# nihofm/volren

Measured on AMD Instinct MI355X. Metric: Msamples/s (pixels x spp / s), volume path tracing, higher is better.
Workload: dtype f32; 1 GPU; BASELINE configs[1] 'c2': smoke.brick, no transfer function, 1024x1024, 1024 spp, seed 42, fov 40; parallelism=1 GPU, 1 fused launch(es)/frame (sample pool budget 64 GiB)

## Files before the change

### volren_amd/csrc/capi.cpp

```cpp
#include "../../include/volren_amd.h"

#include <algorithm>
#include <cmath>
#include <cstring>
#include <filesystem>
#include <functional>
#include <iostream>
#include <stdexcept>
#include <memory>
#include <string>
#include <vector>

#include "imageio.h"
#include "renderer.h"
#include "sharded.h"
#include "vr_device.h"
#include "vr_math_probe.h"

struct vr_renderer {
    vr::RendererHIP impl;
    int device = 0;
};

struct vr_sharded {
// ... 242 lines not shown
    return guard([&] {
        auto& R = r->impl;
        const std::string n = name;
        if (n == "sample") { R.sample = v; R.drop_tile_samples(); }
        else if (n == "sppx") R.sppx = v;
        else if (n == "seed") R.seed = v;
        else if (n == "bounces") R.bounces = v;
        else if (n == "show_environment") R.show_environment = v != 0;
        else if (n == "tonemapping") R.tonemapping = v != 0;
        else if (n == "integrator") R.integrator = v;
        else if (n == "fast_math") R.fast_math = v != 0;
        else if (n == "variance") { if (v < 0 || v > 1) throw std::runtime_error("variance: 0 (off) or 1 (keep the per-pixel second moments)"); R.variance = v; }
        else if (n == "denoise_iterations") {
            if (v < 0 || v > vr::kDenoiseMaxIterations) throw std::runtime_error("denoise_iterations must be in [0, 10]");
            R.denoise_iterations = v;
        }
        else if (n == "denoise_moments") R.set_denoise_moments(v);
        else if (n == "denoise_resolve") R.set_denoise_resolve(v);
        else if (n == "denoise_layers") R.set_denoise_layers(v);
        else if (n == "coalesce_trace") { R.flush_pending(); R.coalesce_trace = v != 0; }
        else if (n == "majorant_layout") { if (v < -1 || v > 1) throw std::runtime_error("majorant_layout: -1 (per grid, chosen at commit), 0 (linear), 1 (4x4x4-cell blocks)"); R.majorant_layout = v; }
        else if (n == "tf_float_atlas") R.tf_float_atlas = v != 0;
        else if (n == "wide_addressing") { if (v < 0 || v > 1) throw std::runtime_error("wide_addressing: 0 (by the tables' sizes), 1 (always the kernels with 64-bit gather addresses)"); R.tuning.wide_addressing = v; }
        else if (n == "gpu_encoder") R.gpu_encoder = v != 0;
        else if (n == "sample_pool_mb") { if (v < 16 || v > 65536) throw std::runtime_error("sample_pool_mb must be in [16, 65536] (item indices of a sub-launch are 32-bit: < 2^32 RGBA32F items)"); R.sample_pool_bytes = (size_t)v << 20; }
        else if (n == "seed_table_mb") {
            if (v < -1 || v > vr::RendererHIP::kSeedTableMaxMb) throw std::runtime_error("seed_table_mb must be in [0, 8192] (0 = no table), or -1 for the default min(4096, sample_pool_mb / 4)");
            R.seed_table_mb = v;
        }
        else if (n == "seed_table_max_samples") { if (v < 0) throw std::runtime_error("seed_table_max_samples must be >= 0 (0 = as many as seed_table_mb holds)"); R.seed_table_max_samples = v; }
        else if (n == "launch_target_ms") { if (v < 0) throw std::runtime_error("launch_target_ms must be >= 0 (0 = no sizing by time)"); R.launch_target_ms = v; }
        else if (n == "expected_skip") { if (v < 0 || v > 1) throw std::runtime_error("expected_skip: 0 (march every step) or 1 (drop the steps of empty space by the clear-distance table)"); R.expected_skip = v; }
        else if (n == "expected_stats") { if (v < 0 || v > 1) throw std::runtime_error("expected_stats: 0 (off) or 1 (the expected-value passes count their work)"); R.expected_stats = v; }
        else if (n == "order_tiles") { if (v < 0 || v > 2) throw std::runtime_error("order_tiles: 0 (never), 1 (tile subsets), 2 (always)"); R.order_tiles = v; }
        else if (n == "grid_frame_counter") {
            if (!R.volume || v < 0 || (size_t)v >= R.volume->n_grid_frames()) throw std::runtime_error("grid_frame_counter out of range");
            R.volume->grid_frame_counter = (size_t)v;
        } else throw std::runtime_error("unknown int parameter: " + n);
    });
}

int vr_get_int(vr_renderer* r, const char* name, int* v) {
    NEED(r);
    if (!name || !v) return fail(VR_ERR_ARG, "null argument");
    return guard([&] {
        auto& R = r->impl;
// ... 2 lines not shown
        else if (n == "sppx") *v = R.sppx;
        else if (n == "seed") *v = R.seed;
        else if (n == "bounces") *v = R.bounces;
        else if (n == "show_environment") *v = R.show_environment ? 1 : 0;
        else if (n == "tonemapping") *v = R.tonemapping ? 1 : 0;
        else if (n == "integrator") *v = R.integrator;
        else if (n == "fast_math") *v = R.fast_math ? 1 : 0;
        else if (n == "variance") *v = R.variance;
        else if (n == "denoise_iterations") *v = R.denoise_iterations;
        else if (n == "denoise_moments") *v = R.denoise_moments;
        else if (n == "denoise_resolve") *v = R.denoise_resolve;
        else if (n == "denoise_layers") *v = R.denoise_layers;
        else if (n == "coalesce_trace") *v = R.coalesce_trace ? 1 : 0;
        else if (n == "majorant_layout") *v = R.majorant_layout;
        else if (n == "majorant_blocked") {
            vr::SceneParams P; R.fill_params(P); *v = P.density.maj_blocked;
        }
        else if (n == "kernel_variant" || n == "kernel_variant_reason") {
            vr::SceneParams P; R.fill_params(P);
            int why = 0; const int variant = vr::pathtrace_variant_of(P, &why);
            *v = n == "kernel_variant" ? variant : why;
        }
        else if (n == "wide_addressing") *v = R.tuning.wide_addressing;
        else if (n == "kernel_wide") {
            vr::SceneParams P; R.fill_params(P);
            *v = (vr::pathtrace_wide_of(R.tuning, P) || vr::pathtrace_variant_of(P, nullptr) >= 2) ? 1 : 0;
        }
        else if (n == "env_div_safe") *v = R.environment && R.environment->cdf_div_safe ? 1 : 0;
        else if (n == "env_compact") *v = R.environment && R.environment->envmap_rgbe ? 1 : 0;
        else if (n == "pending_samples") *v = R.pending_samples();
        else if (n == "tf_float_atlas") *v = R.tf_float_atlas ? 1 : 0;
        else if (n == "gpu_encoder") *v = R.gpu_encoder ? 1 : 0;
        else if (n == "sample_pool_mb") *v = (int)(R.sample_pool_bytes >> 20);
        else if (n == "seed_table_mb") *v = R.seed_table_budget_mb();
        else if (n == "seed_table_max_samples") *v = R.seed_table_max_samples;
        else if (n == "seed_table_samples") *v = R.seed_table_samples();
        else if (n == "seed_table_fills") *v = R.seed_table_fills();
        else if (n == "launch_target_ms") *v = R.launch_target_ms;
        else if (n == "expected_skip") *v = R.expected_skip;
        else if (n == "expected_stats") *v = R.expected_stats;
        else if (n == "order_tiles") *v = R.order_tiles;
        else if (n == "grid_frame_counter") *v = R.volume ? (int)R.volume->grid_frame_counter : 0;
        else if (n == "n_grid_frames") *v = R.volume ? (int)R.volume->n_grid_frames() : 0;
        else if (n == "last_launches") *v = R.last_launches;
        else if (n == "adaptive_rounds") *v = R.adaptive_rounds;
        else if (n == "width") *v = R.resolution.x;
// ... 497 lines not shown
```

### volren_amd/csrc/renderer.cpp

```cpp
#include "renderer.h"

#include <algorithm>
#include <cfloat>
#include <cmath>
#include <cstdlib>
#include <cstring>
#include <iostream>
#include <mutex>

#include "vr_adaptive.h"
#include "vr_device.h"
#include "vr_math.h"
#include "vr_probe.h"

namespace vr {

mat3 Camera::view_inverse() const {
    const vec3 f = normalize(dir);
    const vec3 s = normalize(cross(f, up));
    const vec3 u = cross(s, f);
    mat3 r(0.0f);
    r.m[0] = s.x; r.m[1] = s.y; r.m[2] = s.z;
    r.m[3] = u.x; r.m[4] = u.y; r.m[5] = u.z;
    r.m[6] = -f.x; r.m[7] = -f.y; r.m[8] = -f.z;
    return r;
}

RendererHIP::~RendererHIP() {
    if (ev0_) (void)hipEventDestroy(ev0_);
    if (ev1_) (void)hipEventDestroy(ev1_);
    for (hipEvent_t e : pt_events_) (void)hipEventDestroy(e);
    if (seed_event_) (void)hipEventDestroy(seed_event_);
}

void RendererHIP::init() {
    int n_dev = 0;
    if (hipGetDeviceCount(&n_dev) != hipSuccess || n_dev == 0)
        throw std::runtime_error("RendererHIP::init: no HIP device available (this renderer has no CPU path)");
    if (!volume) volume = std::make_shared<Volume>();
    if (!environment) {
        const float white[3] = { 1.f, 1.f, 1.f };
        environment = std::make_shared<Environment>(white, 1, 1);
    }
    if (!ev0_) { VR_HIP(hipEventCreate(&ev0_)); VR_HIP(hipEventCreate(&ev1_)); }
    if (!status_) {
        status_ = make_device_buffer(16 * sizeof(uint32_t));
        VR_HIP(hipMemset(status_->get(), 0, 16 * sizeof(uint32_t)));
    }
    if (!color && resolution.x > 0 && resolution.y > 0) resize((uint32_t)resolution.x, (uint32_t)resolution.y);
}

void RendererHIP::resize(uint32_t w, uint32_t h) {
    if (w == 0 || h == 0) throw std::runtime_error("RendererHIP::resize: empty framebuffer");
    pending_n_ = 0; pending_ = LaunchInputs{};
    resolution = { (int)w, (int)h };
    color = make_device_buffer((size_t)w * h * 4 * sizeof(float));
    display.reset();
    sized_ = Sized{};
    drop_tile_samples();
    drop_seed_table();
    VR_HIP(hipMemset(color->get(), 0, color->size_bytes()));
    if (!tiles_host_.empty()) set_tiles(tiles_host_);
}

void RendererHIP::reset() { sample = 0; drop_tile_samples(); }

static void check_grid_bytes(size_t bytes, const char* what, const int32_t nb[3]);
constexpr size_t kBlockedMajorantBricks = (size_t)1 << 18;
static size_t brick_records(const BrickGridHIP& g);

// ... 381 lines not shown
    for (size_t k = 0; k < ids.size(); ++k) ordered[k] = ids[(size_t)perm[k]];
    return ordered;
}

const int32_t* RendererHIP::tile_order(const SceneParams& P, const std::vector<int32_t>& ids, int n_tiles) {
    const Uniforms& u = P.u;
    uint64_t key = 1469598103934665603ull;
    auto mix = [&key](const void* p, size_t nbytes) { const uint8_t* b = static_cast<const uint8_t*>(p); for (size_t i = 0; i < nbytes; ++i) { key ^= b[i]; key *= 1099511628211ull; } };
    mix(u.cam_pos, sizeof u.cam_pos); mix(u.cam_transform, sizeof u.cam_transform); mix(&P.cam_z, sizeof P.cam_z);
    mix(u.vol_bb_min, sizeof u.vol_bb_min); mix(u.vol_bb_max, sizeof u.vol_bb_max); mix(u.resolution, sizeof u.resolution); mix(&n_tiles, sizeof n_tiles);
    if (!ids.empty()) mix(ids.data(), ids.size() * sizeof(int32_t));
    key = key ? key : 1;
    if (order_dev_ && order_key_ == key && order_dev_->size_bytes() == (size_t)n_tiles * sizeof(int32_t)) return order_dev_->as<int32_t>();
    const std::vector<int32_t> ordered = costliest_first(P, ids, n_tiles);
    ensure_buffer(order_dev_, ordered.size() * sizeof(int32_t));
    order_dev_->upload(ordered.data(), ordered.size() * sizeof(int32_t), stream);
    order_key_ = key;
    return order_dev_->as<int32_t>();
}

bool RendererHIP::LaunchInputs::same_launch_as(const LaunchInputs& o) const {
    return memcmp(&P, &o.P, sizeof P) == 0 && frame == o.frame && maj.density_scale == o.maj.density_scale && maj.tf_version == o.maj.tf_version &&
           maj.wl == o.maj.wl && maj.ww == o.maj.ww && maj.blocked == o.maj.blocked && memcmp(tuning.thr, o.tuning.thr, sizeof tuning.thr) == 0 && tuning.stats == o.tuning.stats &&
           tuning.samples_per_unit == o.tuning.samples_per_unit && tuning.blocks_per_cu == o.tuning.blocks_per_cu && tuning.wide_addressing == o.tuning.wide_addressing && order_tiles == o.order_tiles &&
           launch_target_ms == o.launch_target_ms && fast_math == o.fast_math && variance == o.variance && sample_pool_bytes == o.sample_pool_bytes && stream == o.stream;
}

void RendererHIP::capture(LaunchInputs& in) {
    if (!color) throw std::runtime_error("RendererHIP::trace: no framebuffer (call resize first)");
    if (integrator == 2 && !transferfunc) throw std::runtime_error("RendererHIP::trace: integrator 2 (direct volume rendering) needs a transfer function");
    if (integrator < 0 || integrator > 3) throw std::runtime_error("RendererHIP::trace: unknown integrator");
    if (fast_math && transferfunc) throw std::runtime_error("RendererHIP::trace: fast_math is not available while a transfer function is bound (it misses the 1e-3 bound there); set fast_math 0");
    if (!volume || volume->grids.empty() || density_grids.empty()) throw std::runtime_error("RendererHIP::trace: no volume committed");
    if (volume->grid_frame_counter >= density_grids.size()) throw std::runtime_error("RendererHIP::trace: grid_frame_counter out of range (commit() after changing the volume)");
    {
        BrickGridHIP& g = density_grids[volume->grid_frame_counter];
        const bool build = transferfunc && tf_float_atlas && !g.dense && g.atlas && g.rng && !g.atlas_f32 && !g.atlas_f32_failed;
        const bool drop = (!transferfunc || !tf_float_atlas) && (g.atlas_f32 || g.atlas_f32_failed);
        if (build || drop) flush_pending();
        if (build) {
            try {
                const size_t n_blocks = g.atlas->size_bytes() / kBrickBlockBytes, want = n_blocks * 512u * sizeof(float);
                auto drop_others = [&] { for (BrickGridHIP& other : density_grids) if (&other != &g) other.atlas_f32.reset(); };
                size_t free_b = 0, total_b = 0;
                if (hipMemGetInfo(&free_b, &total_b) != hipSuccess) { (void)hipGetLastError(); free_b = ~(size_t)0; }
                if (want > free_b / 2) drop_others();
                try { g.atlas_f32 = make_device_buffer(want); }
// ... 111 lines not shown
            if (first > 0) sized_.moments_n = -1;
        }
        moments = sized_.moments->as<float>();
        sized_.moments_n = first == 0 ? n : (sized_.moments_n == first ? first + n : -1);
    } else {
        sized_.moments_n = -1;
    }
    if (!keep_timing_) {
        VR_HIP(hipEventRecord(ev0_, stream));
        last_launches = 0;
        pt_events_used_ = 0;
    }
    for (int done = 0; done < n;) {
        ++last_launches;
        const int m = probe > 0 ? probe : std::min(per_launch, n - done);
        hipEvent_t eb = nullptr, ee = nullptr;
        if (pt_kernel) {
            while (pt_events_.size() < pt_events_used_ + 2) { hipEvent_t e; VR_HIP(hipEventCreate(&e)); pt_events_.push_back(e); }
            eb = pt_events_[pt_events_used_]; ee = pt_events_[pt_events_used_ + 1];
            pt_events_used_ += 2;
        }
        int seed_samples = 0;
        const uint32_t* seed_table = pathtrace_reads_seed_table(in.tuning, P) ? seed_table_for(P, first + done, m, stream, &seed_samples) : nullptr;
        launch_pathtrace(in.tuning, P, color->as<float>(), pool_->as<float>(), workspace_->as<float>(), status_->as<uint32_t>() + 1, tiles, n_tiles, first + 1 + done, m, status_->as<uint32_t>(), stream, in.fast_math != 0, eb, ee, moments,
                         seed_table, seed_samples);
        VR_HIP(hipGetLastError());
        done += m;
        if (pt_kernel) { rate_pending_samples_ = px_samples * (double)m; rate_pending_key_ = key; }
        if (probe > 0) {
            probe = 0;
            harvest_rate(true);
            per_launch = cap_by_rate(per_launch);
        }
    }
    VR_HIP(hipEventRecord(ev1_, stream));
    timing_pending_ = true;
}

int RendererHIP::seed_table_samples_for(long long mb, int w, int h) {
    if (mb <= 0 || w <= 0 || h <= 0) return 0;
    const long long per_sample = (long long)tile_count(w, h) * 256 * (long long)sizeof(uint32_t);
    return (int)std::min<long long>((mb << 20) / per_sample, 1 << 24);
}

void RendererHIP::drop_seed_table() {
    seed_table_.reset();
    seed_cap_ = seed_filled_ = 0;
// ... 626 lines not shown
```

### volren_amd/csrc/renderer.h

```cpp
#pragma once

#include <algorithm>
#include <memory>
#include <string>
#include <vector>

#include "devmem.h"
#include "environment.h"
#include "grids.h"
#include "transferfunc.h"
#include "vr_device.h"
#include "vr_scene.h"

namespace vr {

struct Camera {
    vec3 pos{ 1.f, 0.f, 1.f };
    vec3 dir = normalize(-pos);
    vec3 up{ 0.f, 1.f, 0.f };
    float fov_degree = 70.f;
    mat3 view_inverse() const;
};

struct BrickGridHIP {
// ... 156 lines not shown
        size_t sample_pool_bytes = 0;
        hipStream_t stream = nullptr;
        std::shared_ptr<Environment> env;
        std::shared_ptr<TransferFunction> tf;
        DeviceBufferPtr keep[5];
        bool same_launch_as(const LaunchInputs& o) const;
    };
    void capture(LaunchInputs& in);
    void submit(const LaunchInputs& in, int first, int n, const int32_t* tiles, int n_tiles);
    void submit_tile_set(const LaunchInputs& in, int first, int n);
    int samples_per_launch(const LaunchInputs& in, int n_tiles) const;
    LaunchInputs pending_;
    int pending_n_ = 0, pending_first_ = 0, pending_cap_ = 0;
    void update_majorants(const LaunchInputs& in, BrickGridHIP& g);
    std::vector<int32_t> tiles_host_;
    DeviceBufferPtr tiles_dev_;
    DeviceBufferPtr order_dev_;
    uint64_t order_key_ = 0;
    std::vector<int32_t> costliest_first(const SceneParams& P, const std::vector<int32_t>& ids, int n_tiles) const;
    const int32_t* tile_order(const SceneParams& P, const std::vector<int32_t>& ids, int n_tiles);
    std::vector<int32_t> tile_n_;
    int tile_n_sample_ = -1;
    bool keep_timing_ = false;
    DeviceBufferPtr status_;
    DeviceBufferPtr pool_;
    DeviceBufferPtr workspace_;
    DeviceBufferPtr seed_table_;
    int seed_cap_ = 0, seed_filled_ = 0, seed_fills_ = 0, seed_budget_mb_ = -1, seed_max_samples_ = 0;
    int seed_key_[3] = { 0, 0, 0 };
    bool seed_failed_ = false;
    hipStream_t seed_stream_ = nullptr;
    hipEvent_t seed_event_ = nullptr;
    void drop_seed_table();
    const uint32_t* seed_table_for(const SceneParams& P, int s0, int n, hipStream_t stream, int* samples);
    DeviceBufferPtr stats_;
    struct Sized {
        DeviceBufferPtr features;
        int pass = 0, rays = 0;
        DeviceBufferPtr moments;
        int moments_n = -1;
        DeviceBufferPtr rs_bg, rs_part, resolved;
        DeviceBufferPtr ly_split, ly_filtered, layer;
        bool layer_valid = false;
        DeviceBufferPtr dn_guide, dn_var[2], dn_color[2];
        DeviceBufferPtr denoised;
        DeviceBufferPtr dn_reject;
// ... 34 lines not shown
```

### volren_amd/csrc/vr_device.h

```cpp
#pragma once

#include <hip/hip_runtime.h>
#include <stdint.h>

#include "vr_denoise.h"
#include "vr_scene.h"
#include "vr_temporal.h"
#include "vr_tiles.h"

namespace vr {

struct PathtraceTuning {
    int32_t thr[8] = { 64, 0, 56, 0, 60, 60, 64, 0 };
    unsigned long long* stats = nullptr;
    int32_t samples_per_unit = 0;
    int32_t blocks_per_cu = 0;
    int32_t wide_addressing = 0;
};
PathtraceTuning default_tuning();
size_t pathtrace_pool_floats(const PathtraceTuning& T, int32_t n_tiles, int32_t n_samples);
size_t pathtrace_workspace_floats();
void launch_pathtrace(const PathtraceTuning& T, const SceneParams& P, float* fb, float* sample_pool, float* workspace, uint32_t* unit_counter, const int32_t* tiles, int32_t n_tiles,
                      int32_t first_sample, int32_t n_samples, uint32_t* status, hipStream_t stream, bool fast_math = false,
                      hipEvent_t ev_kernel_begin = nullptr, hipEvent_t ev_kernel_end = nullptr,
                      float* moments = nullptr,
                      const uint32_t* seed_table = nullptr, int32_t seed_samples = 0);
constexpr uint32_t kFeatureLostStatus = 4u;
void launch_features(const SceneParams& P, const int32_t* tiles, int32_t n_tiles, int32_t spp, float* out, uint32_t* status, hipStream_t stream);
constexpr int32_t kExpectedMaxRays = 4;
void launch_features_expected(const SceneParams& P, const int32_t* tiles, int32_t n_tiles, int32_t rays, float* out, hipStream_t stream,
                              const ClearTable* clear = nullptr, unsigned long long* stats = nullptr);
enum PathtraceVariantReason : int {
    VR_VARIANT_INTEGRATOR = 1,
    VR_VARIANT_ENV_DIVISION = 2,
    VR_VARIANT_DENSITY_SCALE = 4,
    VR_VARIANT_GRID_FORMS = 8
};
int pathtrace_variant_of(const SceneParams& P, int* why);
bool pathtrace_reads_seed_table(const PathtraceTuning& T, const SceneParams& P);
bool pathtrace_wide_of(const PathtraceTuning& T, const SceneParams& P);
void launch_denoise_prepare(const float* moments, const float* features, int32_t W, int32_t H, int32_t n, float vscale, const int32_t* counts, float* v, float* guide,
                            hipStream_t stream);
void launch_denoise_atrous(const float* cin, const float* vin, const float* guide, int32_t W, int32_t H, int32_t step, const DenoiseSigma& sg,
                           float* cout, float* vout, hipStream_t stream);
// ... 51 lines not shown
```

### volren_amd/csrc/vr_launch.hip

```cpp
#include <hip/hip_runtime.h>

#include <algorithm>
#include <cstdlib>
#include <map>
#include <mutex>
#include <stdexcept>
#include <string>

#include "vr_device.h"
#include "vr_expected.h"
#include "vr_pathtrace.h"

namespace vr {

template <int INTEGRATOR>
__global__ void __launch_bounds__(256)
item_kernel(const SceneParams P, float* __restrict__ sbuf, const LaunchDesc D) {
    const uint32_t per_unit = (uint32_t)(D.spu * 64);
    const uint32_t g = blockIdx.x * 256u + threadIdx.x;
    const uint32_t u = g / per_unit, item = g - u * per_unit;
    if (u >= D.n_units) return;
    const WorkUnit wu = make_unit(D, P.u.resolution[0], u, sbuf);
    if ((int32_t)item >= wu.n_items) return;
    const int32_t px = wu.px0 + (int32_t)(item & 7u), py = wu.py0 + (int32_t)((item >> 3) & 7u);
// ... 179 lines not shown
    }
    return variant;
}

static int resident_blocks(const PathtraceTuning& T, int mode, int wide, int variant, bool tf, bool stats) {
    int dev = 0, cus = 0;
    if (hipGetDevice(&dev) != hipSuccess) return 1024;
    static std::mutex mu;
    static std::map<uint32_t, std::pair<int, int>> cache;
    const uint32_t key = ((uint32_t)dev << 8) | ((uint32_t)wide << 6) | ((uint32_t)mode << 5) | ((uint32_t)variant << 2) | (tf ? 2u : 0u) | (stats ? 1u : 0u);
    std::pair<int, int> v;
    {
        std::lock_guard<std::mutex> lock(mu);
        auto it = cache.find(key);
        if (it == cache.end()) {
            if (hipDeviceGetAttribute(&cus, hipDeviceAttributeMultiprocessorCount, dev) != hipSuccess || cus <= 0) cus = 256;
            it = cache.emplace(key, std::make_pair(cus, kPtOccupancy[mode][wide][variant](tf, stats))).first;
        }
        v = it->second;
    }
    const int per_cu = T.blocks_per_cu > 0 ? T.blocks_per_cu : v.second;
    return std::min(v.first * per_cu, kMaxWorkgroups * 4 / kWgWaves);
}

size_t pathtrace_workspace_floats() { return kColdMainFloats + (size_t)kMaxWorkgroups * 4u * (size_t)kColdSideWaveFloats; }

void launch_pathtrace(const PathtraceTuning& T, const SceneParams& P, float* fb, float* sample_pool, float* workspace, uint32_t* unit_counter, const int32_t* tiles, int32_t n_tiles,
                      int32_t first_sample, int32_t n_samples, uint32_t* status, hipStream_t stream, bool fast_math, hipEvent_t ev_kernel_begin, hipEvent_t ev_kernel_end,
                      float* moments, const uint32_t* seed_table, int32_t seed_samples) {
    if (n_tiles <= 0 || n_samples <= 0) return;
    SchedParams S;
    for (int i = 0; i < ST_COUNT; ++i) S.thr[i] = T.thr[i];
    LaunchDesc D;
    D.tiles = tiles; D.n_tiles = n_tiles; D.first_sample = first_sample; D.n_samples = n_samples;
    const int variant = pathtrace_variant(P);
    D.spu = std::min(n_samples, samples_per_unit(T, variant));
    const int32_t chunks = (n_samples + D.spu - 1) / D.spu;
    if ((uint64_t)chunks * (uint64_t)n_tiles * 4u * (uint64_t)(D.spu * 64) > 0xFFFFFFFFull)
        throw std::runtime_error("launch_pathtrace: " + std::to_string(n_tiles) + " tiles x " + std::to_string(n_samples) + " samples do not fit the 32-bit item index of one launch");
    D.n_units = (uint32_t)chunks * (uint32_t)n_tiles * 4u;
    D.chunks = (uint32_t)chunks;
    D.seg_len = (D.n_units + kQueueSegments - 1u) / kQueueSegments;
    D.unit_counter = unit_counter;
    SeedTable seeds;
    seeds.table = seed_samples > 0 ? seed_table : nullptr;
    seeds.cap = seed_samples;
    seeds.n_tiles = tile_count(P.u.resolution[0], P.u.resolution[1]);
    S.max_iters = kMaxIdleIters;
    if (S.thr[ST_COLLIDE] <= 0) S.thr[ST_COLLIDE] = (P.u.use_tf || P.u.has_emission) ? 32 : 24;
    const bool tf = P.u.use_tf != 0, stats = T.stats != nullptr;
    const int mode = fast_math ? 1 : 0, wide = pathtrace_wide_of(T, P) ? 1 : 0;
    const int blocks = resident_blocks(T, mode, wide, variant, tf, stats);
    const uint32_t groups_needed = (D.n_units + (uint32_t)kWgWaves - 1u) / (uint32_t)kWgWaves;
    const dim3 grid((unsigned)std::min<uint32_t>((uint32_t)blocks, groups_needed > 0 ? groups_needed : 1u)), block(256);
    if (P.u.integrator == 3 || (P.u.integrator == 2 && P.u.use_tf)) {
        const uint64_t items = (uint64_t)D.n_units * (uint64_t)(D.spu * 64);
        const auto integrate = P.u.integrator == 2 ? item_kernel<2> : item_kernel<3>;
        hipLaunchKernelGGL(integrate, dim3((unsigned)((items + 255) / 256)), block, 0, stream, P, sample_pool, D);
    } else {
        (void)hipMemsetAsync(unit_counter, 0, kQueueSegments * sizeof(uint32_t), stream);
        if (ev_kernel_begin) (void)hipEventRecord(ev_kernel_begin, stream);
        kPtLaunch[mode][wide][variant](tf, stats, grid.x, stream, &P, sample_pool, workspace, &D, &S, status, T.stats, &seeds);
        if (ev_kernel_end) (void)hipEventRecord(ev_kernel_end, stream);
    }
    const auto accumulate = moments ? accumulate_kernel<true> : accumulate_kernel<false>;
    hipLaunchKernelGGL(accumulate, dim3((unsigned)n_tiles), block, 0, stream, sample_pool, fb, moments, tiles, n_tiles, P.u.resolution[0], P.u.resolution[1],
                       first_sample, n_samples, D.spu);
}

}
```

### volren_amd/csrc/vr_pathtrace.h

```cpp
#pragma once

#include <hip/hip_runtime.h>

#include <type_traits>

#include "vr_tiles.h"
#include "vr_trace.h"

namespace vr {

struct SchedParams {
    int32_t thr[ST_COUNT];
    uint32_t max_iters;
};

constexpr uint32_t kQueueSegments = 8u;
constexpr uint32_t kMaxIdleIters = 1u << 26;
constexpr uint64_t kMaxIdleTicks = 7200000000ull;
struct LaunchDesc {
    const int32_t* tiles;
    int32_t n_tiles, first_sample, n_samples, spu;
    uint32_t n_units, chunks, seg_len;
    uint32_t* unit_counter;
};
struct SeedTable {
    const uint32_t* table;
    int32_t cap, n_tiles;
};

__device__ __forceinline__ WorkUnit make_unit(const LaunchDesc& D, int32_t W, uint32_t j, float* sbuf) {
    const uint32_t rem = j / D.chunks, chunk = j - rem * D.chunks;
    const uint32_t slot = rem >> 2, sub = rem & 3u;
    const TilePixel q = wave_tiled_pixel(D.tiles ? D.tiles[slot] : (int32_t)slot, sub * 64u, W);
    WorkUnit wu;
    wu.px0 = q.px;
    wu.py0 = q.py;
    wu.first_sample = D.first_sample + (int32_t)chunk * D.spu;
    wu.n_items = min(D.spu, D.n_samples - (int32_t)chunk * D.spu) * 64;
    wu.base = pool_slot<uint32_t>(chunk, D.n_tiles, slot, sub, D.spu, 0u, 0u);
// ... 9 lines not shown
#endif
#ifndef VR_PRIO_HOT
#define VR_PRIO_HOT 1
#endif
#ifndef VR_PRIO_EVENTS
#define VR_PRIO_EVENTS 0
#endif

typedef __attribute__((address_space(1))) uint32_t SeedGlobal;
template <class K, bool STATS> constexpr int seed_request_point() {
#ifdef VR_SEED_REQ
    return VR_SEED_REQ;
#else
    if (K::emission != 0 || K::global != 0 || K::dense != 0 || STATS) return -1;
    return K::tf ? 0 : 2;
#endif
}

template <class K, bool STATS> constexpr bool collide_tail_early() {
#ifdef VR_COLLIDE_EARLY
    return K::global == 0 && VR_COLLIDE_EARLY != 0;
#else
    return !K::tf && K::global == 0 && K::emission == 0 && K::dense == 0 && K::a32 && !VR_FAST_DEVICE && !STATS;
#endif
}

constexpr int32_t kWgWaves = 4;
constexpr int32_t kLdsPerWorkgroup = 163840 / 16 * kWgWaves;
constexpr int32_t kLutLdsEntries = 256;

enum PoolStack : int32_t { Q_READY = 0, Q_NEE = 1, Q_POST = 2, Q_ESC = 3, Q_FREE = 4, Q_COUNT = 5 };

template <class K> constexpr bool lazy_emission() { return K::emission == 1; }
template <class K> constexpr int32_t hot_stride() { return lazy_emission<K>() ? 15 : 12; }
constexpr int32_t HOT_EL = 12;
template <class K> constexpr int32_t pool_slots() {
#ifdef VR_NSLOT
    return VR_NSLOT;
#else
    const int32_t shared = K::tf ? kLutLdsEntries * 16 + 16 : kWgWaves * 256;
    const int32_t n = (kLdsPerWorkgroup - shared) / kWgWaves / (hot_stride<K>() * 4 + Q_COUNT);
    return n > 192 ? 192 : n;
#endif
}
constexpr int32_t NSLOT = 192;
constexpr int32_t HOT_COL = 4;
// ... 310 lines not shown
        VR_SECTION(0);
#if !VR_STAT_SCHED
        if (STATS_T) { stat_add(26, (uint32_t)popc(wave_ballot(slot >= 0))); stat_add(27, (uint32_t)cnt_ready); stat_add(28, (uint32_t)cnt_nee); stat_add(29, (uint32_t)cnt_post); stat_add(30, (uint32_t)cnt_esc); stat_add(31, (uint32_t)cnt_free); }
#endif
#ifndef VR_HOT_PAIRS
#define VR_HOT_PAIRS 4
#endif
        constexpr int kHotPairs = VR_HOT_PAIRS;

#ifndef VR_HOT_PAIR_MIN
#define VR_HOT_PAIR_MIN 44
#endif
#ifndef VR_DRAIN
#define VR_DRAIN 0
#endif
        const uint64_t holds_path = wave_ballot(slot >= 0);
#ifndef VR_CLEAN_FORMS
#define VR_CLEAN_FORMS 1
#endif
        constexpr bool kCleanForms = VR_CLEAN_FORMS != 0;
        const bool all_clean = kCleanForms && (holds_path & wave_ballot((int32_t)f2u(l.far) < 0)) == 0ull;
        auto hot_pair = [&](auto clean_tag, const int hot_rep_) __attribute__((always_inline)) -> bool {
            constexpr bool CLEAN = decltype(clean_tag)::value;
            if (hot_rep_ > 0 && popc_s(holds_path & wave_ballot((uint32_t)(l.state - ST_MARCH) < 2u)) < (VR_DRAIN && exhausted ? 1 : VR_HOT_PAIR_MIN)) return false;
            if (STATS_T) t_blk = (uint32_t)__builtin_readcyclecounter();
            const bool is_m = slot >= 0 && l.state == ST_MARCH;
            MarchIO mio;
            march_idle(mio);
            if (is_m) march_prep<K::dense, K::majb, CLEAN>(l, P, mio);
            if constexpr (K::maj_reuse) march_load_reuse<K::tf, K::a32>(P, mio, l);
            else march_load<K::tf, K::a32>(P, mio);
            asm volatile("" : "+v"(mio.maj1), "+v"(mio.maj2));
            if (is_m) march_finish<K::tf, K::maj_reuse, CLEAN>(l, P, mio);
            if (STATS) { const int32_t nm = popc(wave_ballot(is_m)); if (nm) { stat_add(2 * ST_MARCH, 1u); stat_add(2 * ST_MARCH + 1, (uint32_t)nm); } }
            if (STATS_T) { const uint32_t t_now = (uint32_t)__builtin_readcyclecounter(); stat_add(18 + ST_MARCH, t_now - t_blk); t_blk = t_now; }
            const bool is_c = slot >= 0 && l.state == ST_COLLIDE;
            const int32_t n_c = popc(holds_path & wave_ballot(l.state == ST_COLLIDE));
            const int32_t n_m = popc(holds_path & wave_ballot(l.state == ST_MARCH));
            const bool run_c = n_c > 0 && n_c >= min(VR_THR_COLLIDE, (n_c + n_m + 1) >> 1);
            if (run_c) {
                CollideIO<K> cio;
                collide_idle<K>(cio);
                const SceneParams& PE = K::emission != 0 ? event_args().P : P;
                const SceneParams& PF = (K::tf && (K::global == 2 || K::emission == 1)) ? event_args().P : P;
                if (is_c) collide_prep<K, CLEAN>(l, PF, PE, cio);
                collide_load<K>(PF, PE, cio);
// ... 50 lines not shown
        const bool want_nee = cnt_nee > 0 && (cnt_nee >= VR_THR_NEE || (hungry && (cnt_nee == big || drain_all)));
        const bool want_post = cnt_post > 0 && (cnt_post >= VR_THR_POST || (hungry && (cnt_post == big || drain_all)));
        const bool want_esc = cnt_esc > 0 && (cnt_esc >= VR_THR_ESC || (hungry && (cnt_esc == big || drain_all)));
        if (want_new || want_nee || want_post || want_esc) {
#if VR_BATCH_REGS
            Hot b;
#else
            const int32_t my_slot = slot;
            const float my_majorant = l.majorant;
            if (my_slot >= 0) { hs.save(l, my_slot); if (emission_on && !l.shadow) { ColdT c = VR_COLD(my_slot); st3(c, C_L, l.eL); } }
            __builtin_amdgcn_wave_barrier();
            Hot& b = l;
#endif
            if (VR_PRIO_EVENTS != VR_PRIO_HOT) __builtin_amdgcn_s_setprio(VR_PRIO_EVENTS);
            constexpr int kSeedReq = seed_request_point<K, STATS>();
            auto pull_unit = [&]() __attribute__((always_inline)) {
                if (cursor != (uint32_t)wu.n_items) return;
                const KernelArgs& E = event_args();
                uint32_t j = 0xFFFFFFFFu;
                while (seg_tries < kQueueSegments) {
                    const uint32_t k = ((blockIdx.x & (kQueueSegments - 1u)) + seg_tries) & (kQueueSegments - 1u);
                    const uint32_t lo = k * E.D.seg_len, hi = min(lo + E.D.seg_len, E.D.n_units);
                    uint32_t v = 0xFFFFFFFFu;
                    if (lo < hi) { if (lane == 0) v = atomicAdd(E.D.unit_counter + k, 1u); v = __builtin_amdgcn_readfirstlane(v); }
                    if (lo < hi && v < hi - lo) { j = lo + v; break; }
                    ++seg_tries;
                }
                if (j == 0xFFFFFFFFu) { exhausted = true; if (STATS_T) t_exhausted = __builtin_amdgcn_s_memrealtime(); }
                else { wu = make_unit(E.D, E.P.u.resolution[0], j, nullptr); cursor = 0u; idle_iters = 0u; t_elapsed = 0u; }
            };
            auto seed_entry = [&](const KernelArgs& E, bool& have) __attribute__((always_inline)) -> uint32_t {
                const uint32_t item = cursor + (uint32_t)lane;
                const uint32_t s = (uint32_t)(wu.first_sample - 1) + (item >> 6);
                have = kSeedReq >= 0 && E.seeds.table != nullptr && item < (uint32_t)wu.n_items && s < (uint32_t)E.seeds.cap;
                return seed_table_index<uint32_t>(s, E.seeds.n_tiles, (uint32_t)tile_of_pixel(wu.px0, wu.py0, E.P.u.resolution[0]), sub_of_pixel(wu.px0, wu.py0), item & 63u);
            };
            auto seed_load = [&](const KernelArgs& E) __attribute__((always_inline)) -> uint32_t {
                uint32_t v = 0u;
                if (kSeedReq >= 0 && E.seeds.table != nullptr) {
                    bool have;
                    const uint32_t i = seed_entry(E, have);
                    v = *(const SeedGlobal*)(E.seeds.table + (size_t)(have ? i : (uint32_t)lane));
                    asm volatile("" ::: "memory");
                }
                return v;
            };
            uint32_t seed_early = 0u;
            auto new_batch = [&]() __attribute__((always_inline)) {
                if (want_new) {
                    if (kSeedReq != 1) pull_unit();
                    n = min(min(64, cnt_free), (int32_t)((uint32_t)wu.n_items - cursor));
                    if (n > 0) {
                        VR_STAT(ST_NEW, n);
                        int32_t bs = -1;
                        const KernelArgs& E = event_args();
                        bool have_seed;
                        seed_entry(E, have_seed);
                        uint32_t table_seed;
                        if (kSeedReq == 1) table_seed = seed_early;
                        else if (kSeedReq == 2) { table_seed = seed_next; have_seed = have_seed && seed_next_valid; }
                        else table_seed = seed_load(E);
                        if (lane < n) {
                            bs = q[Q_FREE * NS + cnt_free - 1 - lane];
                            hot_init(b);
                            ColdT c = VR_COLD(bs);
                            do_new<K, ColdT, kLazyEm>(b, c, E.P, wu, cursor + (uint32_t)lane, have_seed, table_seed);
                            hs.save_new(b, bs);
                            if (kLazyEm) hs.save_first_radiance(v3{ 0.0f, 0.0f, 0.0f }, bs);
                        }
                        cnt_free -= n;
                        cursor += (uint32_t)n;
                        VR_ROUTE_B(bs);
                        VR_STAT_END(ST_NEW);
                    }
                    if (kSeedReq == 2) { pull_unit(); seed_next = seed_load(event_args()); seed_next_valid = true; }
                }
            };
            if (kSeedReq == 1 && want_new) { pull_unit(); seed_early = seed_load(event_args()); }
            if (want_esc) {
                n = min(64, cnt_esc);
                VR_STAT(ST_ESCAPE, n);
                int32_t bs = -1;
                if (lane < n) { bs = q[Q_ESC * NS + cnt_esc - 1 - lane]; hs.load(b, bs); if (kLazyEm && b.first) b.eL = hs.load_first_radiance(bs); }
                if (kItemInRegs) b.item = item_fetch(banks, lane, bs);
                if (lane < n) {
                    const ColdT c = VR_COLD(b.first ? 0 : bs);
                    const KernelArgs& E = event_args();
                    WorkUnit w; w.out = E.sbuf;
                    do_escape<ColdT, kItemInRegs, kLazyEm, kWorld>(b, c, E.P, w);
                }
                cnt_esc -= n;
                VR_ROUTE_B(bs);
                VR_STAT_END(ST_ESCAPE);
            }
            if (want_post) {
                n = min(64, cnt_post);
                VR_STAT(ST_POSTNEE, n);
                int32_t bs = -1;
                if (lane < n) { bs = q[Q_POST * NS + cnt_post - 1 - lane]; hs.load(b, bs); }
                if (kShleInRegs) b.shle = shle_fetch(banks, lane, bs);
                if (kItemInRegs) b.item = item_fetch(banks, lane, bs);
                if (lane < n) {
                    ColdT c = VR_COLD(bs);
                    const KernelArgs& E = event_args();
                    WorkUnit w; w.out = E.sbuf;
                    do_postnee<K, ColdT, kShleInRegs, kItemInRegs>(b, c, E.P, w);
                    hs.save(b, bs);
                }
                cnt_post -= n;
                VR_ROUTE_B(bs);
                VR_STAT_END(ST_POSTNEE);
            }
            if constexpr (kSeedReq < 0) {
                if (want_new) {
                    if (cursor == (uint32_t)wu.n_items) {
                        const KernelArgs& E = event_args();
                        uint32_t j = 0xFFFFFFFFu;
                        while (seg_tries < kQueueSegments) {
                            const uint32_t k = ((blockIdx.x & (kQueueSegments - 1u)) + seg_tries) & (kQueueSegments - 1u);
                            const uint32_t lo = k * E.D.seg_len, hi = min(lo + E.D.seg_len, E.D.n_units);
                            uint32_t v = 0xFFFFFFFFu;
                            if (lo < hi) { if (lane == 0) v = atomicAdd(E.D.unit_counter + k, 1u); v = __builtin_amdgcn_readfirstlane(v); }
                            if (lo < hi && v < hi - lo) { j = lo + v; break; }
                            ++seg_tries;
                        }
                        if (j == 0xFFFFFFFFu) { exhausted = true; if (STATS_T) t_exhausted = __builtin_amdgcn_s_memrealtime(); }
                        else { wu = make_unit(E.D, E.P.u.resolution[0], j, nullptr); cursor = 0u; idle_iters = 0u; t_elapsed = 0u; }
                    }
                    n = min(min(64, cnt_free), (int32_t)((uint32_t)wu.n_items - cursor));
                    if (n > 0) {
                        VR_STAT(ST_NEW, n);
                        int32_t bs = -1;
                        if (lane < n) {
                            bs = q[Q_FREE * NS + cnt_free - 1 - lane];
                            hot_init(b);
                            ColdT c = VR_COLD(bs);
                            do_new<K, ColdT, kLazyEm>(b, c, event_args().P, wu, cursor + (uint32_t)lane);
                            hs.save_new(b, bs);
                            if (kLazyEm) hs.save_first_radiance(v3{ 0.0f, 0.0f, 0.0f }, bs);
                        }
                        cnt_free -= n;
                        cursor += (uint32_t)n;
                        VR_ROUTE_B(bs);
                        VR_STAT_END(ST_NEW);
                    }
// ... 68 lines not shown
```

### volren_amd/csrc/vr_trace.h

```cpp
#pragma once

#include <type_traits>

#include "vr_math.h"
#include "vr_scene.h"

#if defined(VR_HOST_TRACE) && !defined(__HIP_DEVICE_COMPILE__)
namespace vr {
enum TraceClass : int32_t { TR_MAJORANT = 0, TR_TAP = 1, TR_ENV_WARP = 2, TR_ENV_TEXEL = 3 };
void host_trace(int32_t cls, const void* table, size_t a, size_t b);
}
#define VR_TRACE(CLS, TABLE, A, B) ::vr::host_trace((CLS), (TABLE), (size_t)(A), (size_t)(B))
#else
#define VR_TRACE(CLS, TABLE, A, B) do { } while (0)
#endif

namespace vr {

enum LaneState : int32_t {
    ST_NEW = 0,
    ST_BEGIN = 1,
    ST_MARCH = 2,
    ST_COLLIDE = 3,
    ST_NEE = 4,
// ... 1124 lines not shown
    const uint32_t n_paths = f2u(q_l.b) + 1u;
    if (n_paths >= (uint32_t)P.u.bounces) { write_sample(wu, ITEM_IN_HOT ? h.item : ldu(c, C_ITEM), L, n_paths); h.state = ST_NEW; return; }
    const float rr = luma(thr);
    if (rr < 0.1f) {
        const float prob = 1.0f - rr;
        if (rng(h.seed) < prob) { write_sample(wu, ITEM_IN_HOT ? h.item : ldu(c, C_ITEM), L, n_paths); h.state = ST_NEW; return; }
        thr = thr / (1.0f - prob);
        if (!WS) { st3(c, C_THR, thr); c.st(C_FPL, fpl_kept); }
    }
    const v3 dir = q_d.a;
    const float s0 = rng(h.seed), s1 = rng(h.seed);
    const v3 sd = sample_phase_hg(dir, P.u.vol_phase_g, s0, s1);
    const float f_p_next = phase_hg(dot(-dir, sd), P.u.vol_phase_g);
    if (WS) {
        st3(c, C_L, L); stu(c, C_NPATHS, n_paths);
        st3(c, C_THR, thr); c.st(C_FP, f_p_next);
    } else {
        st3(c, C_L, L); stu(c, C_NPATHS, n_paths);
        st3(c, C_DIR, sd); c.st(C_FP, f_p_next);
    }
    begin_segment<K>(h, P, q_p.a, sd, 0);
}

template <class Cold, bool ITEM_IN_HOT = false, bool FIRST_L_IN_HOT = false, bool WS = false>
VR_HD void do_escape(Hot& h, const Cold& c, const SceneParams& P, const WorkUnit& wu) {
    const bool first = h.first != 0;
    v3 L = ld3(c, C_L), thr = ld3(c, C_THR), dir = ld3(c, C_DIR);
    uint32_t n_paths = ldu(c, C_NPATHS), item = ITEM_IN_HOT ? h.item : ldu(c, C_ITEM);
    const float f_p = c.ld(C_FP);
    v3 Le_early = v3{ 0.0f, 0.0f, 0.0f };
    if (WS && P.u.show_environment > 0) Le_early = lookup_environment(P, h.wdir);
    const v3 L_first = FIRST_L_IN_HOT ? h.eL : v3{ 0.0f, 0.0f, 0.0f };
    L = v3{ first ? L_first.x : L.x, first ? L_first.y : L.y, first ? L_first.z : L.z };
    thr = v3{ first ? 1.0f : thr.x, first ? 1.0f : thr.y, first ? 1.0f : thr.z };
    if (WS) dir = h.wdir;
    else dir = v3{ first ? h.ipos.x : dir.x, first ? h.ipos.y : dir.y, first ? h.ipos.z : dir.z };
    n_paths = first ? 0u : n_paths;
    item = first ? f2u(h.Tr) : item;
    h.first = 0;
    if (P.u.show_environment > 0) {
        const v3 Le = WS ? Le_early : lookup_environment(P, dir);
        float mis = 1.0f;
        if (n_paths > 0u) {
            const float avg_w = env_average_importance(P);
            const float pdf_env = (luma(Le) / avg_w) * kInv4Pi;
            mis = power_heuristic(f_p, pdf_env);
        }
        L = L + (thr * mis) * Le;
// ... 234 lines not shown
```

### volren_amd/renderer.py

```python
import ctypes as C

import numpy as np

from . import _lib

_INT_FIELDS = ("sample", "sppx", "seed", "bounces", "show_environment", "tonemapping", "integrator", "grid_frame_counter",
               "sample_pool_mb", "gpu_encoder", "fast_math", "tf_float_atlas", "launch_target_ms", "order_tiles", "coalesce_trace", "majorant_layout",
               "variance", "denoise_iterations", "denoise_moments", "denoise_resolve", "denoise_layers", "wide_addressing", "seed_table_mb", "seed_table_max_samples",
               "expected_skip", "expected_stats")
_FLOAT_FIELDS = {"tonemap_exposure": 1, "tonemap_gamma": 1, "albedo": 3, "phase": 1, "density_scale": 1,
                 "emission_scale": 1, "vol_clip_min": 3, "vol_clip_max": 3, "env_strength": 1, "env_transform": 9,
                 "tf_window_left": 1, "tf_window_width": 1, "cam_pos": 3, "cam_dir": 3, "cam_up": 3, "cam_fov": 1,
                 "volume_transform": 16, "denoise_sigma": 5, "denoise_alpha": 1, "denoise_reject": 1}


def _f32(a):
    return np.ascontiguousarray(a, dtype=np.float32)


class Renderer:

    def __init__(self, width, height, device=0, _borrowed=None):
        object.__setattr__(self, "_h", None)
        L = _lib.load()
        object.__setattr__(self, "_owned", _borrowed is None)
        if _borrowed is None:
            h = C.c_void_p()
            _lib.check(L.vr_create(C.byref(h), int(device), int(width), int(height)))
        else:
            h = C.c_void_p(_borrowed)
        object.__setattr__(self, "_h", h)
# ... 528 lines not shown
```

Measured before the change: 5792 Msamples/s.

## Finish all-miss new-path batches in place and pad work-queue head counters

When every lane of a wave's new-path batch misses the volume, the kernel now writes the environment sample directly and does not claim pool slots or go through the scheduler. A specialised escape path with the first-bounce values fixed is added for this case. Separately, the per-segment work-unit atomic counters are spaced 1024 words apart so they no longer share cache lines. The cost is a larger status buffer, an extra wave ballot per batch, and more code in the persistent kernel.

```diff
diff --git a/volren_amd/csrc/capi.cpp b/volren_amd/csrc/capi.cpp
--- a/volren_amd/csrc/capi.cpp
+++ b/volren_amd/csrc/capi.cpp
@@ -288,6 +288,8 @@
         else if (n == "majorant_layout") { if (v < -1 || v > 1) throw std::runtime_error("majorant_layout: -1 (per grid, chosen at commit), 0 (linear), 1 (4x4x4-cell blocks)"); R.majorant_layout = v; }
         else if (n == "tf_float_atlas") R.tf_float_atlas = v != 0;
         else if (n == "wide_addressing") { if (v < 0 || v > 1) throw std::runtime_error("wide_addressing: 0 (by the tables' sizes), 1 (always the kernels with 64-bit gather addresses)"); R.tuning.wide_addressing = v; }
+        else if (n == "inline_miss") { if (v < 0 || v > 1) throw std::runtime_error("inline_miss: 0 (every new path takes a pool slot), 1 (a batch of new paths that all miss the volume ends in place)"); R.tuning.inline_miss = v; }
+        else if (n == "samples_per_unit") { if (v < 0 || v > 8) throw std::runtime_error("samples_per_unit: 0 (per kernel variant) or 1..8 samples of a pixel tile per work unit"); R.tuning.samples_per_unit = v; }
         else if (n == "gpu_encoder") R.gpu_encoder = v != 0;
         else if (n == "sample_pool_mb") { if (v < 16 || v > 65536) throw std::runtime_error("sample_pool_mb must be in [16, 65536] (item indices of a sub-launch are 32-bit: < 2^32 RGBA32F items)"); R.sample_pool_bytes = (size_t)v << 20; }
         else if (n == "seed_table_mb") {
@@ -336,6 +338,8 @@
             *v = n == "kernel_variant" ? variant : why;
         }
         else if (n == "wide_addressing") *v = R.tuning.wide_addressing;
+        else if (n == "inline_miss") *v = R.tuning.inline_miss;
+        else if (n == "samples_per_unit") *v = R.tuning.samples_per_unit;
         else if (n == "kernel_wide") {
             vr::SceneParams P; R.fill_params(P);
             *v = (vr::pathtrace_wide_of(R.tuning, P) || vr::pathtrace_variant_of(P, nullptr) >= 2) ? 1 : 0;
diff --git a/volren_amd/csrc/renderer.cpp b/volren_amd/csrc/renderer.cpp
--- a/volren_amd/csrc/renderer.cpp
+++ b/volren_amd/csrc/renderer.cpp
@@ -44,8 +44,8 @@
     }
     if (!ev0_) { VR_HIP(hipEventCreate(&ev0_)); VR_HIP(hipEventCreate(&ev1_)); }
     if (!status_) {
-        status_ = make_device_buffer(16 * sizeof(uint32_t));
-        VR_HIP(hipMemset(status_->get(), 0, 16 * sizeof(uint32_t)));
+        status_ = make_device_buffer((kStatusWords + pathtrace_queue_words()) * sizeof(uint32_t));
+        VR_HIP(hipMemset(status_->get(), 0, (kStatusWords + pathtrace_queue_words()) * sizeof(uint32_t)));
     }
     if (!color && resolution.x > 0 && resolution.y > 0) resize((uint32_t)resolution.x, (uint32_t)resolution.y);
 }
@@ -473,7 +473,7 @@
 bool RendererHIP::LaunchInputs::same_launch_as(const LaunchInputs& o) const {
     return memcmp(&P, &o.P, sizeof P) == 0 && frame == o.frame && maj.density_scale == o.maj.density_scale && maj.tf_version == o.maj.tf_version &&
            maj.wl == o.maj.wl && maj.ww == o.maj.ww && maj.blocked == o.maj.blocked && memcmp(tuning.thr, o.tuning.thr, sizeof tuning.thr) == 0 && tuning.stats == o.tuning.stats &&
-           tuning.samples_per_unit == o.tuning.samples_per_unit && tuning.blocks_per_cu == o.tuning.blocks_per_cu && tuning.wide_addressing == o.tuning.wide_addressing && order_tiles == o.order_tiles &&
+           tuning.samples_per_unit == o.tuning.samples_per_unit && tuning.blocks_per_cu == o.tuning.blocks_per_cu && tuning.wide_addressing == o.tuning.wide_addressing && tuning.inline_miss == o.tuning.inline_miss && order_tiles == o.order_tiles &&
            launch_target_ms == o.launch_target_ms && fast_math == o.fast_math && variance == o.variance && sample_pool_bytes == o.sample_pool_bytes && stream == o.stream;
 }
 
@@ -631,7 +631,7 @@
         }
         int seed_samples = 0;
         const uint32_t* seed_table = pathtrace_reads_seed_table(in.tuning, P) ? seed_table_for(P, first + done, m, stream, &seed_samples) : nullptr;
-        launch_pathtrace(in.tuning, P, color->as<float>(), pool_->as<float>(), workspace_->as<float>(), status_->as<uint32_t>() + 1, tiles, n_tiles, first + 1 + done, m, status_->as<uint32_t>(), stream, in.fast_math != 0, eb, ee, moments,
+        launch_pathtrace(in.tuning, P, color->as<float>(), pool_->as<float>(), workspace_->as<float>(), status_->as<uint32_t>() + kStatusWords, tiles, n_tiles, first + 1 + done, m, status_->as<uint32_t>(), stream, in.fast_math != 0, eb, ee, moments,
                          seed_table, seed_samples);
         VR_HIP(hipGetLastError());
         done += m;
diff --git a/volren_amd/csrc/renderer.h b/volren_amd/csrc/renderer.h
--- a/volren_amd/csrc/renderer.h
+++ b/volren_amd/csrc/renderer.h
@@ -202,6 +202,7 @@
     std::vector<int32_t> tile_n_;
     int tile_n_sample_ = -1;
     bool keep_timing_ = false;
+    static constexpr size_t kStatusWords = 1024;
     DeviceBufferPtr status_;
     DeviceBufferPtr pool_;
     DeviceBufferPtr workspace_;
diff --git a/volren_amd/csrc/vr_device.h b/volren_amd/csrc/vr_device.h
--- a/volren_amd/csrc/vr_device.h
+++ b/volren_amd/csrc/vr_device.h
@@ -16,10 +16,12 @@
     int32_t samples_per_unit = 0;
     int32_t blocks_per_cu = 0;
     int32_t wide_addressing = 0;
+    int32_t inline_miss = 1;
 };
 PathtraceTuning default_tuning();
 size_t pathtrace_pool_floats(const PathtraceTuning& T, int32_t n_tiles, int32_t n_samples);
 size_t pathtrace_workspace_floats();
+size_t pathtrace_queue_words();
 void launch_pathtrace(const PathtraceTuning& T, const SceneParams& P, float* fb, float* sample_pool, float* workspace, uint32_t* unit_counter, const int32_t* tiles, int32_t n_tiles,
                       int32_t first_sample, int32_t n_samples, uint32_t* status, hipStream_t stream, bool fast_math = false,
                       hipEvent_t ev_kernel_begin = nullptr, hipEvent_t ev_kernel_end = nullptr,
diff --git a/volren_amd/csrc/vr_launch.hip b/volren_amd/csrc/vr_launch.hip
--- a/volren_amd/csrc/vr_launch.hip
+++ b/volren_amd/csrc/vr_launch.hip
@@ -225,6 +225,8 @@
     const int per_cu = T.blocks_per_cu > 0 ? T.blocks_per_cu : v.second;
     return std::min(v.first * per_cu, kMaxWorkgroups * 4 / kWgWaves);
 }
+
+size_t pathtrace_queue_words() { return kQueueHeadWords; }
 
 size_t pathtrace_workspace_floats() { return kColdMainFloats + (size_t)kMaxWorkgroups * 4u * (size_t)kColdSideWaveFloats; }
 
@@ -250,6 +252,7 @@
     seeds.cap = seed_samples;
     seeds.n_tiles = tile_count(P.u.resolution[0], P.u.resolution[1]);
     S.max_iters = kMaxIdleIters;
+    S.inline_miss = T.inline_miss;
     if (S.thr[ST_COLLIDE] <= 0) S.thr[ST_COLLIDE] = (P.u.use_tf || P.u.has_emission) ? 32 : 24;
     const bool tf = P.u.use_tf != 0, stats = T.stats != nullptr;
     const int mode = fast_math ? 1 : 0, wide = pathtrace_wide_of(T, P) ? 1 : 0;
@@ -261,7 +264,7 @@
         const auto integrate = P.u.integrator == 2 ? item_kernel<2> : item_kernel<3>;
         hipLaunchKernelGGL(integrate, dim3((unsigned)((items + 255) / 256)), block, 0, stream, P, sample_pool, D);
     } else {
-        (void)hipMemsetAsync(unit_counter, 0, kQueueSegments * sizeof(uint32_t), stream);
+        (void)hipMemsetAsync(unit_counter, 0, kQueueHeadWords * sizeof(uint32_t), stream);
         if (ev_kernel_begin) (void)hipEventRecord(ev_kernel_begin, stream);
         kPtLaunch[mode][wide][variant](tf, stats, grid.x, stream, &P, sample_pool, workspace, &D, &S, status, T.stats, &seeds);
         if (ev_kernel_end) (void)hipEventRecord(ev_kernel_end, stream);
diff --git a/volren_amd/csrc/vr_pathtrace.h b/volren_amd/csrc/vr_pathtrace.h
--- a/volren_amd/csrc/vr_pathtrace.h
+++ b/volren_amd/csrc/vr_pathtrace.h
@@ -12,9 +12,15 @@
 struct SchedParams {
     int32_t thr[ST_COUNT];
     uint32_t max_iters;
+    int32_t inline_miss;
 };
 
 constexpr uint32_t kQueueSegments = 8u;
+#ifndef VR_QUEUE_HEAD_STRIDE
+#define VR_QUEUE_HEAD_STRIDE 1024
+#endif
+constexpr uint32_t kQueueHeadStride = VR_QUEUE_HEAD_STRIDE;
+constexpr size_t kQueueHeadWords = (size_t)kQueueSegments * kQueueHeadStride;
 constexpr uint32_t kMaxIdleIters = 1u << 26;
 constexpr uint64_t kMaxIdleTicks = 7200000000ull;
 struct LaunchDesc {
@@ -70,6 +76,14 @@
     return K::global == 0 && VR_COLLIDE_EARLY != 0;
 #else
     return !K::tf && K::global == 0 && K::emission == 0 && K::dense == 0 && K::a32 && !VR_FAST_DEVICE && !STATS;
+#endif
+}
+
+template <class K, bool STATS> constexpr bool inline_miss() {
+#ifdef VR_INLINE_MISS
+    return seed_request_point<K, STATS>() >= 0 && VR_INLINE_MISS != 0;
+#else
+    return seed_request_point<K, STATS>() >= 0 && !(K::tf && VR_FAST_DEVICE);
 #endif
 }
 
@@ -426,6 +440,7 @@
         const bool all_clean = kCleanForms && (holds_path & wave_ballot((int32_t)f2u(l.far) < 0)) == 0ull;
         auto hot_pair = [&](auto clean_tag, const int hot_rep_) __attribute__((always_inline)) -> bool {
             constexpr bool CLEAN = decltype(clean_tag)::value;
+            if (inline_miss<K, STATS>() && hot_rep_ == 0 && (holds_path & wave_ballot((uint32_t)(l.state - ST_MARCH) < 2u)) == 0ull) return false;
             if (hot_rep_ > 0 && popc_s(holds_path & wave_ballot((uint32_t)(l.state - ST_MARCH) < 2u)) < (VR_DRAIN && exhausted ? 1 : VR_HOT_PAIR_MIN)) return false;
             if (STATS_T) t_blk = (uint32_t)__builtin_readcyclecounter();
             const bool is_m = slot >= 0 && l.state == ST_MARCH;
@@ -522,7 +537,7 @@
                     const uint32_t k = ((blockIdx.x & (kQueueSegments - 1u)) + seg_tries) & (kQueueSegments - 1u);
                     const uint32_t lo = k * E.D.seg_len, hi = min(lo + E.D.seg_len, E.D.n_units);
                     uint32_t v = 0xFFFFFFFFu;
-                    if (lo < hi) { if (lane == 0) v = atomicAdd(E.D.unit_counter + k, 1u); v = __builtin_amdgcn_readfirstlane(v); }
+                    if (lo < hi) { if (lane == 0) v = atomicAdd(E.D.unit_counter + k * kQueueHeadStride, 1u); v = __builtin_amdgcn_readfirstlane(v); }
                     if (lo < hi && v < hi - lo) { j = lo + v; break; }
                     ++seg_tries;
                 }
@@ -548,32 +563,76 @@
             uint32_t seed_early = 0u;
             auto new_batch = [&]() __attribute__((always_inline)) {
                 if (want_new) {
-                    if (kSeedReq != 1) pull_unit();
-                    n = min(min(64, cnt_free), (int32_t)((uint32_t)wu.n_items - cursor));
-                    if (n > 0) {
-                        VR_STAT(ST_NEW, n);
-                        int32_t bs = -1;
-                        const KernelArgs& E = event_args();
-                        bool have_seed;
-                        seed_entry(E, have_seed);
-                        uint32_t table_seed;
-                        if (kSeedReq == 1) table_seed = seed_early;
-                        else if (kSeedReq == 2) { table_seed = seed_next; have_seed = have_seed && seed_next_valid; }
-                        else table_seed = seed_load(E);
-                        if (lane < n) {
-                            bs = q[Q_FREE * NS + cnt_free - 1 - lane];
+                    if constexpr (!inline_miss<K, STATS>()) {
+                        if (kSeedReq != 1) pull_unit();
+                        n = min(min(64, cnt_free), (int32_t)((uint32_t)wu.n_items - cursor));
+                        if (n > 0) {
+                            VR_STAT(ST_NEW, n);
+                            int32_t bs = -1;
+                            const KernelArgs& E = event_args();
+                            bool have_seed;
+                            seed_entry(E, have_seed);
+                            uint32_t table_seed;
+                            if (kSeedReq == 1) table_seed = seed_early;
+                            else if (kSeedReq == 2) { table_seed = seed_next; have_seed = have_seed && seed_next_valid; }
+                            else table_seed = seed_load(E);
+                            if (lane < n) {
+                                bs = q[Q_FREE * NS + cnt_free - 1 - lane];
+                                hot_init(b);
+                                ColdT c = VR_COLD(bs);
+                                do_new<K, ColdT, kLazyEm>(b, c, E.P, wu, cursor + (uint32_t)lane, have_seed, table_seed);
+                                hs.save_new(b, bs);
+                                if (kLazyEm) hs.save_first_radiance(v3{ 0.0f, 0.0f, 0.0f }, bs);
+                            }
+                            cnt_free -= n;
+                            cursor += (uint32_t)n;
+                            VR_ROUTE_B(bs);
+                            VR_STAT_END(ST_NEW);
+                        }
+                        if (kSeedReq == 2) { pull_unit(); seed_next = seed_load(event_args()); seed_next_valid = true; }
+                    } else {
+                        if (kSeedReq != 1) pull_unit();
+                        n = min(min(64, cnt_free), (int32_t)((uint32_t)wu.n_items - cursor));
+                        bool asked = false;
+                        if (n > 0) {
+                            VR_STAT(ST_NEW, n);
+                            int32_t bs = -1;
+                            const KernelArgs& E = event_args();
+                            bool have_seed;
+                            seed_entry(E, have_seed);
+                            uint32_t table_seed;
+                            if (kSeedReq == 1) table_seed = seed_early;
+                            else if (kSeedReq == 2) { table_seed = seed_next; have_seed = have_seed && seed_next_valid; }
+                            else table_seed = seed_load(E);
                             hot_init(b);
-                            ColdT c = VR_COLD(bs);
-                            do_new<K, ColdT, kLazyEm>(b, c, E.P, wu, cursor + (uint32_t)lane, have_seed, table_seed);
-                            hs.save_new(b, bs);
-                            if (kLazyEm) hs.save_first_radiance(v3{ 0.0f, 0.0f, 0.0f }, bs);
+                            if (lane < n) {
+                                bs = q[Q_FREE * NS + cnt_free - 1 - lane];
+                                ColdT c = VR_COLD(bs);
+                                do_new<K, ColdT, kLazyEm>(b, c, E.P, wu, cursor + (uint32_t)lane, have_seed, table_seed);
+                            }
+                            const bool ended = b.state == ST_NEW || (b.state == ST_ESCAPE && b.first != 0);
+                            if (wave_ballot(!ended) == 0ull && E.S.inline_miss != 0) {
+                                cursor += (uint32_t)n;
+                                idle_iters = 0u; t_elapsed = 0u;
+                                if (kSeedReq == 2) { pull_unit(); seed_next = seed_load(event_args()); seed_next_valid = true; asked = true; }
+                                if (lane < n && b.state == ST_ESCAPE) {
+                                    const ColdT c = VR_COLD(0);
+                                    WorkUnit w; w.out = E.sbuf;
+                                    do_escape<ColdT, kItemInRegs, kLazyEm, kWorld, true>(b, c, E.P, w);
+                                }
+                            } else {
+                                if (lane < n) {
+                                    hs.save_new(b, bs);
+                                    if (kLazyEm) hs.save_first_radiance(v3{ 0.0f, 0.0f, 0.0f }, bs);
+                                }
+                                cnt_free -= n;
+                                cursor += (uint32_t)n;
+                                VR_ROUTE_B(bs);
+                            }
+                            VR_STAT_END(ST_NEW);
                         }
-                        cnt_free -= n;
-                        cursor += (uint32_t)n;
-                        VR_ROUTE_B(bs);
-                        VR_STAT_END(ST_NEW);
+                        if (kSeedReq == 2 && !asked) { pull_unit(); seed_next = seed_load(event_args()); seed_next_valid = true; }
                     }
-                    if (kSeedReq == 2) { pull_unit(); seed_next = seed_load(event_args()); seed_next_valid = true; }
                 }
             };
             if (kSeedReq == 1 && want_new) { pull_unit(); seed_early = seed_load(event_args()); }
@@ -620,7 +679,7 @@
                             const uint32_t k = ((blockIdx.x & (kQueueSegments - 1u)) + seg_tries) & (kQueueSegments - 1u);
                             const uint32_t lo = k * E.D.seg_len, hi = min(lo + E.D.seg_len, E.D.n_units);
                             uint32_t v = 0xFFFFFFFFu;
-                            if (lo < hi) { if (lane == 0) v = atomicAdd(E.D.unit_counter + k, 1u); v = __builtin_amdgcn_readfirstlane(v); }
+                            if (lo < hi) { if (lane == 0) v = atomicAdd(E.D.unit_counter + k * kQueueHeadStride, 1u); v = __builtin_amdgcn_readfirstlane(v); }
                             if (lo < hi && v < hi - lo) { j = lo + v; break; }
                             ++seg_tries;
                         }
diff --git a/volren_amd/csrc/vr_trace.h b/volren_amd/csrc/vr_trace.h
--- a/volren_amd/csrc/vr_trace.h
+++ b/volren_amd/csrc/vr_trace.h
@@ -1170,8 +1170,22 @@
     begin_segment<K>(h, P, q_p.a, sd, 0);
 }
 
-template <class Cold, bool ITEM_IN_HOT = false, bool FIRST_L_IN_HOT = false, bool WS = false>
+template <class Cold, bool ITEM_IN_HOT = false, bool FIRST_L_IN_HOT = false, bool WS = false, bool KNOWN_FIRST = false>
 VR_HD void do_escape(Hot& h, const Cold& c, const SceneParams& P, const WorkUnit& wu) {
+    if constexpr (KNOWN_FIRST) {
+        v3 L = FIRST_L_IN_HOT ? h.eL : v3{ 0.0f, 0.0f, 0.0f };
+        const v3 thr = v3{ 1.0f, 1.0f, 1.0f }, dir = WS ? h.wdir : h.ipos;
+        const uint32_t item = f2u(h.Tr);
+        h.first = 0;
+        if (P.u.show_environment > 0) {
+            const v3 Le = lookup_environment(P, dir);
+            const float mis = 1.0f;
+            L = L + (thr * mis) * Le;
+        }
+        write_sample(wu, item, L, 0u);
+        h.state = ST_NEW;
+        return;
+    }
     const bool first = h.first != 0;
     v3 L = ld3(c, C_L), thr = ld3(c, C_THR), dir = ld3(c, C_DIR);
     uint32_t n_paths = ldu(c, C_NPATHS), item = ITEM_IN_HOT ? h.item : ldu(c, C_ITEM);
diff --git a/volren_amd/renderer.py b/volren_amd/renderer.py
--- a/volren_amd/renderer.py
+++ b/volren_amd/renderer.py
@@ -6,7 +6,7 @@
 
 _INT_FIELDS = ("sample", "sppx", "seed", "bounces", "show_environment", "tonemapping", "integrator", "grid_frame_counter",
                "sample_pool_mb", "gpu_encoder", "fast_math", "tf_float_atlas", "launch_target_ms", "order_tiles", "coalesce_trace", "majorant_layout",
-               "variance", "denoise_iterations", "denoise_moments", "denoise_resolve", "denoise_layers", "wide_addressing", "seed_table_mb", "seed_table_max_samples",
+               "variance", "denoise_iterations", "denoise_moments", "denoise_resolve", "denoise_layers", "wide_addressing", "inline_miss", "samples_per_unit", "seed_table_mb", "seed_table_max_samples",
                "expected_skip", "expected_stats")
 _FLOAT_FIELDS = {"tonemap_exposure": 1, "tonemap_gamma": 1, "albedo": 3, "phase": 1, "density_scale": 1,
                  "emission_scale": 1, "vol_clip_min": 3, "vol_clip_max": 3, "env_strength": 1, "env_transform": 9,
```

After: 5815 Msamples/s (median of 6 runs). No clear change (+0.4%).
